# Wionerlol/MultimodalEmotionRecognition

Measured on AMD Instinct MI355X. Metric: 3s-clip train steps/sec (B=32, xattn fusion) at 1/2/4/8 MI355X, higher is better.
Workload: dtype bf16; 1 GPU; ResNet18 + WavLM-base (frozen) + xattn fusion train step (fwd+bwd+Adam); per_gpu_batch=32, global_batch=32, frames=8, image=112, audio_samples=48000, parallelism=dp1

## Files before the change

multimodalemotionrecognition_amd/csrc/conv.hip:

```cpp
#include "conv_common.h"
#include "mer.h"

MER_CT_BUFFER(mer_ct, 512 * 64)
MER_CT_BUFFER(mer_ctp, 4096 * 8)
#define CT(k) CT_AT(mer_ct_buf, k)
#define CTP(k) CTP_AT(mer_ctp_buf, k)

namespace {

template <bool DGRAD>
__device__ __forceinline__ u32x4 conv_a_chunk(const ConvGeom& g, int n, int oh, int ow, bool rowok, int kk, int tap,
                                              int c, int r, int s) {
  u32x4 v = {0u, 0u, 0u, 0u};
  if (!rowok || kk >= g.Kred) return v;
  int ih, iw;
  if (!DGRAD) {
    ih = oh * g.st - g.pad + r;
    iw = ow * g.st - g.pad + s;
  } else {
    const int th = oh + g.pad - r, tw = ow + g.pad - s;
    if (th < 0 || tw < 0) return v;
    if (g.st == 1) {
      ih = th;
      iw = tw;
    } else if (g.st == 2) {
      if ((th | tw) & 1) return v;
      ih = th >> 1;
      iw = tw >> 1;
    } else {
      if ((th % g.st) || (tw % g.st)) return v;
      ih = th / g.st;
      iw = tw / g.st;
    }
  }
  if (ih < 0 || ih >= g.IH || iw < 0 || iw >= g.IW) return v;
  return *reinterpret_cast<const u32x4*>(g.X + (((long)n * g.IH + ih) * g.IW + iw) * g.IC + c);
}

template <bool DGRAD, int BM_, int BN_>
__global__ __launch_bounds__(256, 2) void conv_kernel(ConvGeom g) {
  constexpr int LDK = CBK + 8;
  constexpr int IT = BM_ / 32, JT = BN_ / 32;
  constexpr int ACH = BM_ * 8 / 256, BCH = BN_ * 8 / 256;
  __shared__ __attribute__((aligned(16))) bf16_t lds[2][(BM_ + BN_) * LDK];
  const int t = threadIdx.x, lane = t & 63, w = t >> 6;
  const int M = g.N * g.OH * g.OW;
  const int nx = (g.Ncols + BN_ - 1) / BN_, ny = (M + BM_ - 1) / BM_;
  int tx, ty;
  xcd_tile(blockIdx.x, nx, nx * ny, tx, ty);
  const int m0 = ty * BM_, n0 = tx * BN_;
  const int wm = (w >> 1) * (BM_ / 2), wn = (w & 1) * (BN_ / 2);
  const int crow = t >> 3, ckc = t & 7;

  int an[ACH], aoh[ACH], aow[ACH];
  bool aok[ACH];
#pragma unroll
  for (int i = 0; i < ACH; ++i) {
    const int m = m0 + crow + 32 * i;
    aok[i] = m < M;
    const int mm = aok[i] ? m : 0;
    an[i] = mm / (g.OH * g.OW);
    const int rem = mm - an[i] * g.OH * g.OW;
    aoh[i] = rem / g.OW;
    aow[i] = rem - aoh[i] * g.OW;
  }
  u32x4 ra[ACH], rb[BCH];
  const float inv_IC = 1.f / g.IC, inv_S = 1.f / g.S;
  auto gload = [&](int k0) {
    const int kk = k0 + ckc * 8;
    const int tap = fdiv(kk, inv_IC), c = kk - tap * g.IC;
    const int r = fdiv(tap, inv_S), s = tap - r * g.S;
#pragma unroll
    for (int i = 0; i < ACH; ++i) ra[i] = conv_a_chunk<DGRAD>(g, an[i], aoh[i], aow[i], aok[i], kk, tap, c, r, s);
#pragma unroll
    for (int i = 0; i < BCH; ++i) {
      const int n = n0 + crow + 32 * i;
      rb[i] = (n < g.Ncols && kk < g.Kred) ? *reinterpret_cast<const u32x4*>(g.Wt + (long)n * g.Kred + kk)
                                            : u32x4{0u, 0u, 0u, 0u};
    }
  };
  auto lstore = [&](int buf) {
#pragma unroll
    for (int i = 0; i < ACH; ++i)
      *reinterpret_cast<u32x4*>(&lds[buf][(crow + 32 * i) * LDK + ckc * 8]) = ra[i];
#pragma unroll
    for (int i = 0; i < BCH; ++i)
      *reinterpret_cast<u32x4*>(&lds[buf][(BM_ + crow + 32 * i) * LDK + ckc * 8]) = rb[i];
  };
  f32x4 acc[IT][JT];
#pragma unroll
  for (int i = 0; i < IT; ++i)
#pragma unroll
    for (int j = 0; j < JT; ++j) acc[i][j] = f32x4{0.f, 0.f, 0.f, 0.f};

  const int nk = (g.Kred + CBK - 1) / CBK;
  gload(0);
  lstore(0);
  __syncthreads();
  for (int kt = 0; kt < nk; ++kt) {
    const int cur = kt & 1;
    if (kt + 1 < nk) gload((kt + 1) * CBK);
#pragma unroll
    for (int s = 0; s < 2; ++s) {
      const int kof = s * 32 + (lane >> 4) * 8;
      bf16x8 af[IT], bfr[JT];
#pragma unroll
      for (int i = 0; i < IT; ++i)
        af[i] = *reinterpret_cast<const bf16x8*>(&lds[cur][(wm + i * 16 + (lane & 15)) * LDK + kof]);
#pragma unroll
      for (int j = 0; j < JT; ++j)
        bfr[j] = *reinterpret_cast<const bf16x8*>(&lds[cur][(BM_ + wn + j * 16 + (lane & 15)) * LDK + kof]);
#pragma unroll
      for (int i = 0; i < IT; ++i)
#pragma unroll
        for (int j = 0; j < JT; ++j) acc[i][j] = __builtin_amdgcn_mfma_f32_16x16x32_bf16(af[i], bfr[j], acc[i][j], 0, 0, 0);
    }
    if (kt + 1 < nk) lstore(cur ^ 1);
    __syncthreads();
  }

#pragma unroll
  for (int j = 0; j < JT; ++j) {
    const int col = n0 + wn + j * 16 + (lane & 15);
    float csum = 0.f, csq = 0.f;
#pragma unroll
    for (int i = 0; i < IT; ++i)
#pragma unroll
      for (int r = 0; r < 4; ++r) {
        const int row = m0 + wm + i * 16 + (lane >> 4) * 4 + r;
        if (row < M && col < g.Ncols) {
          float v = acc[i][j][r];
          if (g.R_) {
            const long ri = (long)row * g.ldy + col;
            if (!g.Rmask || bf2f(g.Rmask[ri]) > 0.f) v += bf2f(g.R_[ri]);
          }
          const bf16_t h = f2bf(v);
          g.Y[(long)row * g.ldy + col] = h;
          const float hv = bf2f(h);
          csum += hv;
          csq += hv * hv;
        }
      }
    if (g.stats) {
      csum += __shfl_xor(csum, 16, 64);
      csum += __shfl_xor(csum, 32, 64);
      csq += __shfl_xor(csq, 16, 64);
      csq += __shfl_xor(csq, 32, 64);
      if ((lane >> 4) == 0 && col < g.Ncols) {
        float* slab = g.stats + (long)ty * g.Ncols * 2;
        atomicAdd(slab + 2 * col, csum);
        atomicAdd(slab + 2 * col + 1, csq);
      }
    }
  }
}


__device__ __forceinline__ int cswz(int row, int c) { return c ^ ((row >> 1) & 7); }
template <int CW>
__device__ __forceinline__ int cswz_k(int row, int c) {
  return CW == 8 ? (c ^ ((row >> 1) & 7)) : (c ^ ((row >> 2) & 3));
}

template <bool DGRAD>
__device__ __forceinline__ const bf16_t* conv_a_src(const ConvGeom& g, int n, int oh, int ow, bool rowok, int kk,
                                                    float inv_IC, float inv_S) {
  const bf16_t* zero = reinterpret_cast<const bf16_t*>(mer_conv_zero16);
  if (!rowok || kk >= g.Kred) return zero;
  const int tap = fdiv(kk, inv_IC), c = kk - tap * g.IC;
  const int r = fdiv(tap, inv_S), s = tap - r * g.S;
  int ih, iw;
  if (!DGRAD) {
    ih = oh * g.st - g.pad + r;
    iw = ow * g.st - g.pad + s;
  } else {
    const int th = oh + g.pad - r, tw = ow + g.pad - s;
    if (th < 0 || tw < 0) return zero;
    if (g.st == 1) {
      ih = th;
      iw = tw;
    } else {
      if ((th | tw) & 1) return zero;
      ih = th >> 1;
      iw = tw >> 1;
    }
  }
  if (ih < 0 || ih >= g.IH || iw < 0 || iw >= g.IW) return zero;
  return g.X + (((long)n * g.IH + ih) * g.IW + iw) * g.IC + c;
}

struct ParClass {
  int ph, pw, Hc, Wc, r0, s0, nr, ns, dh0, dw0;
};

__device__ __forceinline__ int par_cls() { return 3 - (int)blockIdx.y; }

__device__ __forceinline__ ParClass par_class(const ConvGeom& g, int cls) {
  ParClass c;
  c.ph = cls >> 1;
  c.pw = cls & 1;
  c.Hc = (g.OH - c.ph + 1) >> 1;
  c.Wc = (g.OW - c.pw + 1) >> 1;
  c.r0 = (c.ph + g.pad) & 1;
  c.s0 = (c.pw + g.pad) & 1;
  c.nr = (g.R - c.r0 + 1) >> 1;
  c.ns = (g.S - c.s0 + 1) >> 1;
  c.dh0 = (c.ph + g.pad - c.r0) >> 1;
  c.dw0 = (c.pw + g.pad - c.s0) >> 1;
  return c;
}

template <int FM, int FN, int WM, int WN>
__device__ __forceinline__ void conv_tile_stats_lane(const ConvGeom& g, const f32x4 (&acc)[FM][FN], int w, int lane,
                                                     int m0, int n0, int M, float (&part)[FN][2]) {
  constexpr int TM = FM * 16, TN = FN * 16;
  const int wr = w / WN, wc = w % WN, fr = lane & 15, fq = lane >> 4;
#pragma unroll
  for (int j = 0; j < FN; ++j) {
    const int col = n0 + wc * TN + j * 16 + fr;
    float csum = 0.f, csq = 0.f;
#pragma unroll
    for (int i = 0; i < FM; ++i)
#pragma unroll
      for (int r = 0; r < 4; ++r) {
        const int row = m0 + wr * TM + i * 16 + fq * 4 + r;
        if (row < M && col < g.Ncols) {
          const float hv = acc[i][j][r];
          csum += hv;
          csq += hv * hv;
        }
      }
    part[j][0] = csum;
    part[j][1] = csq;
  }
}

template <int FN, int WM, int WN>
__device__ __forceinline__ void conv_stats_finish(const ConvGeom& g, float (&part)[FN][2], float* red, int w, int lane,
                                                  int n0, long stat_row) {
  constexpr int TN = FN * 16;
  const int wr = w / WN, wc = w % WN, fr = lane & 15, fq = lane >> 4;
#pragma unroll
  for (int j = 0; j < FN; ++j)
#pragma unroll
    for (int q = 0; q < 2; ++q) {
      part[j][q] += __shfl_xor(part[j][q], 16, 64);
      part[j][q] += __shfl_xor(part[j][q], 32, 64);
    }
  lds_barrier();
  if (wr > 0 && fq == 0)
#pragma unroll
    for (int j = 0; j < FN; ++j) {
      red[((wr * WN + wc) * FN * 16 + j * 16 + fr) * 2] = part[j][0];
      red[((wr * WN + wc) * FN * 16 + j * 16 + fr) * 2 + 1] = part[j][1];
    }
  lds_barrier();
  if (wr == 0 && fq == 0) {
    float* slab = g.stats + stat_row * g.Ncols * 2;
#pragma unroll
    for (int j = 0; j < FN; ++j) {
      const int col = n0 + wc * TN + j * 16 + fr;
      float t0 = part[j][0], t1 = part[j][1];
#pragma unroll
      for (int q = 1; q < WM; ++q) {
        t0 += red[((q * WN + wc) * FN * 16 + j * 16 + fr) * 2];
        t1 += red[((q * WN + wc) * FN * 16 + j * 16 + fr) * 2 + 1];
      }
      if (col < g.Ncols) {
        slab[2 * col] = t0;
        slab[2 * col + 1] = t1;
      }
    }
  }
}

template <int FM, int FN, int WM, int WN>
__device__ __forceinline__ void conv_tile_stats(const ConvGeom& g, const f32x4 (&acc)[FM][FN], float* red, int w,
                                                int lane, int m0, int n0, int M, long stat_row) {
  float part[FN][2];
  conv_tile_stats_lane<FM, FN, WM, WN>(g, acc, w, lane, m0, n0, M, part);
  conv_stats_finish<FN, WM, WN>(g, part, red, w, lane, n0, stat_row);
}

typedef __attribute__((ext_vector_type(8))) float f32x8;
template <int FN>
struct EpiAcc {
  f32x8 sA, sB, sC;
  float fs[FN][2];
  __device__ void zero() {
    sA = sB = sC = f32x8{0.f, 0.f, 0.f, 0.f, 0.f, 0.f, 0.f, 0.f};
#pragma unroll
    for (int j = 0; j < FN; ++j) fs[j][0] = fs[j][1] = 0.f;
  }
};
struct EpiNoAcc {};

template <int FM, int FN, int WAVE_FLOATS>
struct EpiGeo {
  static constexpr int TM = FM * 16, TN = FN * 16, LDT = TN + 4;
  static constexpr int GI0 = WAVE_FLOATS / (16 * LDT);
  static constexpr int GI = GI0 < FM ? GI0 : FM;
  static constexpr int LPR = TN / 8, RPP = 64 / LPR;
  static constexpr int PPG = (GI * 16 + RPP - 1) / RPP;
  static constexpr int NP = ((FM + GI - 1) / GI) * PPG;
};

template <int NP>
struct EpiPre {
  u32x4 r[NP], m[NP], bm[NP], x[NP], x2[NP];
  float mu[8], rs[8], mu2[8], rs2[8];
};
struct EpiNone {};

template <bool DGRAD, int FM, int FN, int WM, int WN, int WAVE_FLOATS, class OutRow, int NP, bool X2 = true>
__device__ __forceinline__ void conv_epilogue_prefetch(const ConvGeom& g, EpiPre<NP>& pre, int w, int lane, int m0,
                                                       int n0, int M, OutRow out_row) {
  using E = EpiGeo<FM, FN, WAVE_FLOATS>;
  static_assert(NP == E::NP, "prefetch pass count");
  const int wr = w / WN, wc = w % WN;
  const int lr = lane / E::LPR, lc = (lane % E::LPR) * 8;
  const int colv = n0 + wc * E::TN + lc;
  const bool cok = colv < g.Ncols;
  const bool do_bnr = DGRAD && g.bnr_red != nullptr;
  const bool has_x2 = X2 && do_bnr && g.bnr_x2 != nullptr;
  const u32x4 z = {0u, 0u, 0u, 0u};
#pragma unroll
  for (int e = 0; e < 8; ++e) {
    const int col = cok ? colv + e : 0;
    pre.mu[e] = do_bnr ? g.bnr_ms[2 * col] : 0.f;
    pre.rs[e] = do_bnr ? g.bnr_ms[2 * col + 1] : 0.f;
    pre.mu2[e] = has_x2 ? g.bnr_ms2[2 * col] : 0.f;
    pre.rs2[e] = has_x2 ? g.bnr_ms2[2 * col + 1] : 0.f;
  }
#pragma unroll
  for (int q = 0; q < NP; ++q) {
    const int i0 = (q / E::PPG) * E::GI, rr = (q % E::PPG) * E::RPP;
    int row = m0 + wr * E::TM + i0 * 16 + rr + lr;
    row = row < M ? row : M - 1;
    const long e0 = out_row(row) * g.ldy + (cok ? colv : 0);
    pre.r[q] = (DGRAD && g.R_) ? *reinterpret_cast<const u32x4*>(g.R_ + e0) : z;
    pre.m[q] = (DGRAD && g.R_ && g.Rmask) ? *reinterpret_cast<const u32x4*>(g.Rmask + e0) : z;
    pre.bm[q] = do_bnr ? *reinterpret_cast<const u32x4*>(g.bnr_mask + e0) : z;
    pre.x[q] = do_bnr ? *reinterpret_cast<const u32x4*>(g.bnr_x + e0) : z;
    pre.x2[q] = has_x2 ? *reinterpret_cast<const u32x4*>(g.bnr_x2 + e0) : z;
  }
}

template <bool DGRAD, int FM, int FN, int WM, int WN, int WAVE_FLOATS, class OutRow, class Pre = EpiNone,
          bool DEFER = false, bool X2 = true, class AccT = EpiNoAcc>
__device__ __forceinline__ void conv_epilogue_vec(const ConvGeom& g, f32x4 (&acc)[FM][FN], float* smemf, int w,
                                                  int lane, int m0, int n0, int M, long red_row_id, long stat_row,
                                                  OutRow out_row, const Pre* pre = nullptr, int ct_slot = -1,
                                                  AccT* accp = nullptr) {
  constexpr bool PREF = !std::is_same<Pre, EpiNone>::value;
  constexpr bool ACC = !std::is_same<AccT, EpiNoAcc>::value;
  using E = EpiGeo<FM, FN, WAVE_FLOATS>;
  constexpr int TM = FM * 16, TN = FN * 16;
  const int wr = w / WN, wc = w % WN, fr = lane & 15, fq = lane >> 4;
  constexpr int LDT = TN + 4;
  constexpr int GI = E::GI;
  static_assert(GI >= 1, "epilogue staging slice too small");
  constexpr int LPR = TN / 8, RPP = 64 / LPR;
  float* wl = smemf + w * WAVE_FLOATS;
  const int lr = lane / LPR, lc = (lane % LPR) * 8;
  const int colv = n0 + wc * TN + lc;
  const bool cok = colv < g.Ncols;
  const bool do_bnr = DGRAD && g.bnr_red != nullptr;
  const bool has_x2 = X2 && do_bnr && g.bnr_x2 != nullptr;
  float mu[8], rs[8], mu2[8], rs2[8];
  float sA[8], sB[8], sC[8];
  constexpr int NPS = DEFER ? E::NP : 1;
  u32x4 pend[NPS];
  long pend_at[NPS];
  bool pend_ok[NPS];
#pragma unroll
  for (int q = 0; q < NPS; ++q) pend_ok[q] = false;
  auto flush = [&]() {
#pragma unroll
    for (int q = 0; q < NPS; ++q)
      if (pend_ok[q]) *reinterpret_cast<u32x4*>(g.Y + pend_at[q]) = pend[q];
  };
#pragma unroll
  for (int e = 0; e < 8; ++e) {
    if constexpr (PREF) {
      mu[e] = pre->mu[e];
      rs[e] = pre->rs[e];
      mu2[e] = pre->mu2[e];
      rs2[e] = pre->rs2[e];
    } else {
      const int col = cok ? colv + e : 0;
      mu[e] = do_bnr ? g.bnr_ms[2 * col] : 0.f;
      rs[e] = do_bnr ? g.bnr_ms[2 * col + 1] : 0.f;
      mu2[e] = has_x2 ? g.bnr_ms2[2 * col] : 0.f;
      rs2[e] = has_x2 ? g.bnr_ms2[2 * col + 1] : 0.f;
    }
    sA[e] = sB[e] = sC[e] = 0.f;
  }
#pragma unroll
  for (int i0 = 0; i0 < FM; i0 += GI) {
#pragma unroll
    for (int ii = 0; ii < GI; ++ii) {
      if (i0 + ii >= FM) break;
#pragma unroll
      for (int j = 0; j < FN; ++j)
#pragma unroll
        for (int r = 0; r < 4; ++r) wl[(ii * 16 + fq * 4 + r) * LDT + j * 16 + fr] = acc[i0 + ii][j][r];
    }
    __builtin_amdgcn_fence(__ATOMIC_RELEASE, "wavefront");
    __builtin_amdgcn_wave_barrier();
    __builtin_amdgcn_fence(__ATOMIC_ACQUIRE, "wavefront");
    const int nrows = (FM - i0 < GI ? FM - i0 : GI) * 16;
#pragma unroll
    for (int rr = 0; rr < GI * 16; rr += RPP) {
      const int rl = rr + lr;
      const int row = m0 + wr * TM + i0 * 16 + rl;
      if (rl < nrows && row < M && cok) {
        const f32x4 lo = *reinterpret_cast<const f32x4*>(&wl[rl * LDT + lc]);
        const f32x4 hi = *reinterpret_cast<const f32x4*>(&wl[rl * LDT + lc + 4]);
        float v[8] = {lo[0], lo[1], lo[2], lo[3], hi[0], hi[1], hi[2], hi[3]};
        const long e0 = out_row(row) * g.ldy + colv;
        const int q = (i0 / GI) * E::PPG + rr / RPP;
        if (DGRAD && g.R_) {
          u32x4 rv, mv;
          if constexpr (PREF) {
            rv = pre->r[q];
            mv = g.Rmask ? pre->m[q] : u32x4{1u, 1u, 1u, 1u};
          } else {
            rv = *reinterpret_cast<const u32x4*>(g.R_ + e0);
            mv = g.Rmask ? *reinterpret_cast<const u32x4*>(g.Rmask + e0) : u32x4{1u, 1u, 1u, 1u};
          }
          const bf16_t* rh = reinterpret_cast<const bf16_t*>(&rv);
          const bf16_t* mh = reinterpret_cast<const bf16_t*>(&mv);
#pragma unroll
          for (int e = 0; e < 8; ++e)
            if (!g.Rmask || bf2f(mh[e]) > 0.f) v[e] += bf2f(rh[e]);
        }
        u32x4 ov;
        bf16_t* oh = reinterpret_cast<bf16_t*>(&ov);
#pragma unroll
        for (int e = 0; e < 8; ++e) {
          oh[e] = f2bf(v[e]);
          v[e] = bf2f(oh[e]);
        }
        if constexpr (DEFER) {
          pend[q] = ov;
          pend_at[q] = e0;
          pend_ok[q] = true;
        } else {
          *reinterpret_cast<u32x4*>(g.Y + e0) = ov;
        }
        if (do_bnr) {
          u32x4 mv, xv, x2v;
          if constexpr (PREF) {
            mv = pre->bm[q];
            xv = pre->x[q];
            x2v = pre->x2[q];
          } else {
            mv = *reinterpret_cast<const u32x4*>(g.bnr_mask + e0);
            xv = *reinterpret_cast<const u32x4*>(g.bnr_x + e0);
            x2v = has_x2 ? *reinterpret_cast<const u32x4*>(g.bnr_x2 + e0) : u32x4{0u, 0u, 0u, 0u};
          }
          const bf16_t* mh = reinterpret_cast<const bf16_t*>(&mv);
          const bf16_t* xh = reinterpret_cast<const bf16_t*>(&xv);
          const bf16_t* x2h = reinterpret_cast<const bf16_t*>(&x2v);
#pragma unroll
          for (int e = 0; e < 8; ++e) {
            const float gv = bf2f(mh[e]) > 0.f ? v[e] : 0.f;
            sA[e] += gv;
            sB[e] += gv * (bf2f(xh[e]) - mu[e]) * rs[e];
            if (has_x2) sC[e] += gv * (bf2f(x2h[e]) - mu2[e]) * rs2[e];
          }
        }
      }
    }
    __builtin_amdgcn_fence(__ATOMIC_RELEASE, "wavefront");
    __builtin_amdgcn_wave_barrier();
    __builtin_amdgcn_fence(__ATOMIC_ACQUIRE, "wavefront");
  }
  if (ct_slot >= 0) CT(ct_slot);
  if constexpr (ACC) {
    if (do_bnr) {
#pragma unroll
      for (int e = 0; e < 8; ++e) {
        accp->sA[e] += sA[e];
        accp->sB[e] += sB[e];
        accp->sC[e] += sC[e];
      }
      flush();
      return;
    }
  }
  if (do_bnr) {
#pragma unroll
  for (int o = LPR; o < 64; o <<= 1)
#pragma unroll
    for (int e = 0; e < 8; ++e) {
      sA[e] += __shfl_xor(sA[e], o, 64);
      sB[e] += __shfl_xor(sB[e], o, 64);
      if (has_x2) sC[e] += __shfl_xor(sC[e], o, 64);
    }
  if (ct_slot >= 0) CT(ct_slot + 3);
  float* red = smemf;
  lds_barrier();
  if (ct_slot >= 0) CT(ct_slot + 4);
  if (wr > 0 && lane < LPR)
#pragma unroll
    for (int e = 0; e < 8; ++e) {
      float* o = red + ((wr * WN + wc) * TN + lc + e) * 3;
      o[0] = sA[e];
      o[1] = sB[e];
      o[2] = sC[e];
    }
  lds_barrier();
  if (wr != 0 || lane >= LPR || !cok) {
    flush();
    return;
  }
#pragma unroll
  for (int e = 0; e < 8; ++e)
#pragma unroll
    for (int q = 1; q < WM; ++q) {
      const float* o = red + ((q * WN + wc) * TN + lc + e) * 3;
      sA[e] += o[0];
      sB[e] += o[1];
      sC[e] += o[2];
    }
  {
    const long slab = red_row_id * g.Ncols * 2 + 2 * colv;
#pragma unroll
    for (int e = 0; e < 8; e += 2) {
      *reinterpret_cast<f32x4*>(g.bnr_red + slab + 2 * e) = f32x4{sA[e], sB[e], sA[e + 1], sB[e + 1]};
      if (g.bnr_red2)
        *reinterpret_cast<f32x4*>(g.bnr_red2 + slab + 2 * e) = f32x4{sA[e], sC[e], sA[e + 1], sC[e + 1]};
    }
  }
  if (ct_slot >= 0) CT(ct_slot + 1);
  flush();
  if (ct_slot >= 0) CT(ct_slot + 2);
  return;
  }
  if (!g.stats) {
    flush();
    return;
  }
#pragma unroll
  for (int i = 0; i < FM; ++i)
#pragma unroll
    for (int j = 0; j < FN; ++j)
#pragma unroll
      for (int r = 0; r < 4; ++r) acc[i][j][r] = bf2f(f2bf(acc[i][j][r]));
  if constexpr (ACC) {
    float part[FN][2];
    conv_tile_stats_lane<FM, FN, WM, WN>(g, acc, w, lane, m0, n0, M, part);
#pragma unroll
    for (int j = 0; j < FN; ++j) {
      accp->fs[j][0] += part[j][0];
      accp->fs[j][1] += part[j][1];
    }
    flush();
    return;
  }
  conv_tile_stats<FM, FN, WM, WN>(g, acc, smemf, w, lane, m0, n0, M, stat_row);
  if (ct_slot >= 0) CT(ct_slot + 1);
  flush();
  if (ct_slot >= 0) CT(ct_slot + 2);
}

template <bool DGRAD, int FM, int FN, int WM, int WN, int WAVE_FLOATS, bool X2 = true>
__device__ __forceinline__ void conv_epilogue_acc_finish(const ConvGeom& g, EpiAcc<FN>& a, float* smemf, int w,
                                                         int lane, int n0, long row_id) {
  if constexpr (DGRAD) {
    if (!g.bnr_red) return;
    using E = EpiGeo<FM, FN, WAVE_FLOATS>;
    constexpr int TN = FN * 16, LPR = E::LPR;
    const int wr = w / WN, wc = w % WN;
    const int lc = (lane % LPR) * 8;
    const int colv = n0 + wc * TN + lc;
    const bool cok = colv < g.Ncols;
    const bool has_x2 = X2 && g.bnr_x2 != nullptr;
#pragma unroll
    for (int o = LPR; o < 64; o <<= 1)
#pragma unroll
      for (int e = 0; e < 8; ++e) {
        a.sA[e] += __shfl_xor(a.sA[e], o, 64);
        a.sB[e] += __shfl_xor(a.sB[e], o, 64);
        if (has_x2) a.sC[e] += __shfl_xor(a.sC[e], o, 64);
      }
    float* red = smemf;
    lds_barrier();
    if (wr > 0 && lane < LPR)
#pragma unroll
      for (int e = 0; e < 8; ++e) {
        float* o = red + ((wr * WN + wc) * TN + lc + e) * 3;
        o[0] = a.sA[e];
        o[1] = a.sB[e];
        o[2] = a.sC[e];
      }
    lds_barrier();
    if (wr != 0 || lane >= LPR || !cok) return;
#pragma unroll
    for (int e = 0; e < 8; ++e)
#pragma unroll
      for (int q = 1; q < WM; ++q) {
        const float* o = red + ((q * WN + wc) * TN + lc + e) * 3;
        a.sA[e] += o[0];
        a.sB[e] += o[1];
        a.sC[e] += o[2];
      }
    const long slab = row_id * g.Ncols * 2 + 2 * colv;
#pragma unroll
    for (int e = 0; e < 8; e += 2) {
      *reinterpret_cast<f32x4*>(g.bnr_red + slab + 2 * e) = f32x4{a.sA[e], a.sB[e], a.sA[e + 1], a.sB[e + 1]};
      if (g.bnr_red2)
        *reinterpret_cast<f32x4*>(g.bnr_red2 + slab + 2 * e) = f32x4{a.sA[e], a.sC[e], a.sA[e + 1], a.sC[e + 1]};
    }
  } else {
    if (!g.stats) return;
    conv_stats_finish<FN, WM, WN>(g, a.fs, smemf, w, lane, n0, row_id);
  }
}

constexpr int conv_pipe_wpe(int nw, int bm, int bn, int stages, bool dgrad, bool par, int lds_bytes = 0) {
  return (nw >= 16 || 2 * lds_bytes > 160 * 1024)
             ? (nw >= 4 ? nw / 4 : 1)
             : nw == 8 ? ((dgrad && (bm == 256 || (!par && bm == 128 && bn == 128 && stages == 3))) ? 2 : 4) : 2;
}
constexpr int conv_pipe_lds(int bm, int bn, int stages, int ks, int kg) {
  return kg * stages * (bm + bn) * ks * 2 > (kg > 1 ? kg * bm * (bn + 4) * 4 : 0)
             ? kg * stages * (bm + bn) * ks * 2
             : kg * bm * (bn + 4) * 4;
}

template <int BM_, int BN_, int NW>
struct KgLayout {
  static constexpr int WM = (NW >= 4 && BM_ / 4 >= 16) ? 4 : (NW >= 2 ? 2 : 1);
  static constexpr int WN = NW / WM;
  static_assert(WM * WN == NW && BM_ % (16 * WM) == 0 && BN_ % (16 * WN) == 0, "split-K epilogue layout");
};

template <bool DGRAD, bool PAR, int BM_, int BN_, int WM = 2, int WN = 2, int STAGES = 2, int KS = 64, bool X2 = true,
          int KG = 1, bool FAST = false>
__global__ __launch_bounds__(64 * WM * WN * KG, conv_pipe_wpe(WM * WN * KG, BM_, BN_, STAGES, DGRAD, PAR,
                                                              conv_pipe_lds(BM_, BN_, STAGES, KS, KG))) void conv_pipe_kernel(ConvGeom g) {
  constexpr int WAVES = WM * WN;
  constexpr int CW = KS / 8, RPG = 64 / CW;
  constexpr int IA = BM_ / RPG / WAVES, IB = BN_ / RPG / WAVES;
  static_assert(IA * RPG * WAVES == BM_ && IB * RPG * WAVES == BN_, "tile rows must split into whole glds pieces");
  static_assert(KS == 64 || KS == 32, "K-tile");
  static_assert(KG == 1 || KG == 2 || KG == 4, "K-groups");
  constexpr int TM = BM_ / WM, TN = BN_ / WN, FM = TM / 16, FN = TN / 16;
  constexpr int BUF = (BM_ + BN_) * KS;
  extern __shared__ __attribute__((aligned(16))) bf16_t smem_all[];
  const int t = threadIdx.x, lane = t & 63, kg = (t >> 6) / WAVES, w = (t >> 6) % WAVES;
  bf16_t* const smem = smem_all + kg * STAGES * BUF;
  ParClass pc{};
  int M, Kr, rowsH, rowsW;
  int Kr0 = 0;
  if (PAR) {
    pc = par_class(g, par_cls());
    M = g.N * pc.Hc * pc.Wc;
    Kr0 = pc.nr * pc.ns * g.IC;
    Kr = Kr0 + ((g.X2 && pc.ph == 0 && pc.pw == 0) ? g.K2 : 0);
    rowsH = pc.Hc;
    rowsW = pc.Wc;
  } else {
    M = g.N * g.OH * g.OW;
    Kr = g.Kred;
    rowsH = g.OH;
    rowsW = g.OW;
  }
  const int nx = (g.Ncols + BN_ - 1) / BN_, ny = (M + BM_ - 1) / BM_;
  if ((int)blockIdx.x >= nx * ny) return;
  CTP(0);
  int tx, ty;
  xcd_tile(blockIdx.x, nx, nx * ny, tx, ty);
  const int m0 = ty * BM_, n0 = tx * BN_;
  const int wr = w / WN, wc = w % WN;

  auto a_row = [&](int j, int& n, int& oh, int& ow, bool& ok) {
    const int m = m0 + (w * IA + j) * RPG + lane / CW;
    ok = m < M;
    const int mm = ok ? m : 0;
    n = mm / (rowsH * rowsW);
    const int rem = mm - n * rowsH * rowsW;
    oh = rem / rowsW;
    ow = rem - oh * rowsW;
  };
  int acl[IA];
#pragma unroll
  for (int j = 0; j < IA; ++j) acl[j] = cswz_k<CW>((w * IA + j) * RPG + lane / CW, lane % CW) * 8;
  int bcl[IB], bn[IB];
  bool bok[IB];
#pragma unroll
  for (int j = 0; j < IB; ++j) {
    const int r = (w * IB + j) * RPG + lane / CW;
    const int n = n0 + r;
    bok[j] = n < g.Ncols;
    bn[j] = bok[j] ? n : 0;
    bcl[j] = cswz_k<CW>(r, lane % CW) * 8;
  }
  const bf16_t* zero = reinterpret_cast<const bf16_t*>(mer_conv_zero16);

  f32x4 acc[FM][FN];
#pragma unroll
  for (int i = 0; i < FM; ++i)
#pragma unroll
    for (int j = 0; j < FN; ++j) acc[i][j] = f32x4{0.f, 0.f, 0.f, 0.f};

  const int fr = lane & 15, fq = lane >> 4;
  const int nk_all = (Kr + KS - 1) / KS;
  const int nkg = (nk_all + KG - 1) / KG, kb = __builtin_amdgcn_readfirstlane(kg * nkg);
  const int nk = nk_all - kb < nkg ? (nk_all - kb > 0 ? nk_all - kb : 0) : nkg;
  const int kofs = kb * KS;
  constexpr int G = IA + IB;
  static_assert(STAGES >= 2 && STAGES <= 4, "ring depth");
  auto k_loop = [&](auto&& stage) {
#pragma unroll
    for (int p = 0; p < STAGES - 1; ++p)
      if (p < nk) stage(p);
    int wslot = STAGES - 1, rslot = 0;
    CTP(1);
    for (int kt = 0; kt < nkg; ++kt) {
      const int left = nk - 1 - kt;
      const int ahead = left < (STAGES - 2) ? left : (STAGES - 2);
      wait_tiles_in_flight<G>(ahead);
      lds_barrier();
      if (kt + STAGES - 1 < nk) stage(wslot);
      wslot = wslot == STAGES - 1 ? 0 : wslot + 1;
      const bf16_t* la = smem + rslot * BUF;
      rslot = rslot == STAGES - 1 ? 0 : rslot + 1;
      if (KG > 1 && kt >= nk) continue;
      const bf16_t* lb = la + BM_ * KS;
#pragma unroll
      for (int s = 0; s < KS / 32; ++s) {
        bf16x8 af[FM], bfr[FN];
#pragma unroll
        for (int i = 0; i < FM; ++i) {
          const int r = wr * TM + i * 16 + fr;
          af[i] = *reinterpret_cast<const bf16x8*>(la + r * KS + cswz_k<CW>(r, s * 4 + fq) * 8);
        }
#pragma unroll
        for (int j = 0; j < FN; ++j) {
          const int r = wc * TN + j * 16 + fr;
          bfr[j] = *reinterpret_cast<const bf16x8*>(lb + r * KS + cswz_k<CW>(r, s * 4 + fq) * 8);
        }
        __builtin_amdgcn_s_setprio(1);
#pragma unroll
        for (int i = 0; i < FM; ++i)
#pragma unroll
          for (int j = 0; j < FN; ++j)
            acc[i][j] = __builtin_amdgcn_mfma_f32_16x16x32_bf16(af[i], bfr[j], acc[i][j], 0, 0, 0);
        __builtin_amdgcn_s_setprio(0);
      }
    }
  };

  if constexpr (FAST) {
    const bool has_ds = PAR && Kr > Kr0;
    constexpr bool NEG = DGRAD || PAR;
    const int nr = PAR ? pc.nr : g.R, ns = PAR ? pc.ns : g.S;
    const bf16_t* fa[IA];
    unsigned fm[IA];
#pragma unroll
    for (int j = 0; j < IA; ++j) {
      int n, oh, ow;
      bool ok;
      a_row(j, n, oh, ow, ok);
      const int h0 = PAR ? oh + pc.dh0 : DGRAD ? oh + g.pad : oh * g.st - g.pad;
      const int w0 = PAR ? ow + pc.dw0 : DGRAD ? ow + g.pad : ow * g.st - g.pad;
      unsigned cm = 0, m = 0;
      for (int si = 0; si < ns; ++si) cm |= (unsigned)((unsigned)(NEG ? w0 - si : w0 + si) < (unsigned)g.IW) << si;
      for (int ri = 0; ri < nr; ++ri)
        if ((unsigned)(NEG ? h0 - ri : h0 + ri) < (unsigned)g.IH) m |= cm << (ri * ns);
      fm[j] = ok ? m : 0u;
      fa[j] = g.X + ((((long)n * g.IH + h0) * g.IW + w0) * g.IC + acl[j]);
    }
    const bf16_t* fb[IB];
#pragma unroll
    for (int j = 0; j < IB; ++j) fb[j] = g.Wt + ((long)bn[j] * g.Kred + bcl[j]);
    int f_ic = g.IC, f_c, f_tap, f_ri, f_si, f_aoff, f_boff;
    bool f_ds = false;
    auto tap_offsets = [&]() {
      const int ao = (f_ri * g.IW + f_si) * g.IC;
      f_aoff = NEG ? -ao : ao;
      f_boff = PAR ? ((pc.r0 + 2 * f_ri) * g.S + pc.s0 + 2 * f_si) * g.IC : f_tap * g.IC;
    };
    auto enter_ds = [&]() {
      f_ds = true;
      f_ic = g.K2;
      f_c = f_tap = f_ri = f_si = f_aoff = f_boff = 0;
#pragma unroll
      for (int j = 0; j < IA; ++j) {
        int n, hh, ww;
        bool ok;
        a_row(j, n, hh, ww, ok);
        fm[j] = ok ? 1u : 0u;
        fa[j] = g.X2 + ((((long)n * g.IH + hh) * g.IW + ww) * g.K2 + acl[j]);
      }
#pragma unroll
      for (int j = 0; j < IB; ++j) fb[j] = g.Wt2 + ((long)bn[j] * g.K2 + bcl[j]);
    };
    if (has_ds && kofs >= Kr0) {
      enter_ds();
      f_c = kofs - Kr0;
    } else {
      f_tap = kofs / g.IC;
      f_c = kofs - f_tap * g.IC;
      f_ri = f_tap / (ns > 0 ? ns : 1);
      f_si = f_tap - f_ri * ns;
      tap_offsets();
    }
    k_loop([&](int buf) {
      bf16_t* la = smem + buf * BUF;
      bf16_t* lb = la + BM_ * KS;
      const unsigned tbit = 1u << (f_tap & 31);
      const long ao = f_aoff + f_c, bo = f_boff + f_c;
#pragma unroll
      for (int j = 0; j < IA; ++j) glds16((fm[j] & tbit) ? fa[j] + ao : zero, la + (w * IA + j) * 512);
#pragma unroll
      for (int j = 0; j < IB; ++j) glds16(bok[j] ? fb[j] + bo : zero, lb + (w * IB + j) * 512);
      f_c += KS;
      if (f_c == f_ic) {
        f_c = 0;
        ++f_tap;
        if (++f_si == ns) {
          f_si = 0;
          ++f_ri;
        }
        tap_offsets();
        if (has_ds && !f_ds && f_tap == nr * ns) enter_ds();
      }
    });
  } else {
    int an[IA], aoh[IA], aow[IA];
    bool aok[IA];
#pragma unroll
    for (int j = 0; j < IA; ++j) a_row(j, an[j], aoh[j], aow[j], aok[j]);
    const bf16_t* pb[IB];
    const bf16_t* pb2[IB];
#pragma unroll
    for (int j = 0; j < IB; ++j) {
      pb[j] = g.Wt + (long)bn[j] * g.Kred;
      pb2[j] = g.Wt2 + (long)bn[j] * g.K2;
    }
    const float inv_IC = 1.f / g.IC, inv_S = 1.f / g.S, inv_ns = PAR ? 1.f / pc.ns : 1.f;
    auto par_a_src = [&](int n, int hh, int ww, bool rowok, int kk) -> const bf16_t* {
      if (!rowok || kk >= Kr) return zero;
      if (kk >= Kr0)
        return g.X2 + (((long)n * g.IH + hh) * g.IW + ww) * g.K2 + (kk - Kr0);
      const int tap = fdiv(kk, inv_IC), c = kk - tap * g.IC;
      const int ri = fdiv(tap, inv_ns), si = tap - ri * pc.ns;
      const int ih = hh + pc.dh0 - ri, iw = ww + pc.dw0 - si;
      if (ih < 0 || ih >= g.IH || iw < 0 || iw >= g.IW) return zero;
      return g.X + (((long)n * g.IH + ih) * g.IW + iw) * g.IC + c;
    };
    auto par_b_off = [&](int kk) -> int {
      const int tap = fdiv(kk, inv_IC), c = kk - tap * g.IC;
      const int ri = fdiv(tap, inv_ns), si = tap - ri * pc.ns;
      return ((pc.r0 + 2 * ri) * g.S + pc.s0 + 2 * si) * g.IC + c;
    };
    int k0 = kofs;
    k_loop([&](int buf) {
      bf16_t* la = smem + buf * BUF;
      bf16_t* lb = la + BM_ * KS;
#pragma unroll
      for (int j = 0; j < IA; ++j) {
        const bf16_t* src = PAR ? par_a_src(an[j], aoh[j], aow[j], aok[j], k0 + acl[j])
                                : conv_a_src<DGRAD>(g, an[j], aoh[j], aow[j], aok[j], k0 + acl[j], inv_IC, inv_S);
        glds16(src, la + (w * IA + j) * 512);
      }
#pragma unroll
      for (int j = 0; j < IB; ++j) {
        const int kk = k0 + bcl[j];
        const bool ok = bok[j] && kk < Kr;
        const bf16_t* src = !PAR ? pb[j] + kk : (kk >= Kr0 ? pb2[j] + (kk - Kr0) : pb[j] + par_b_off(kk));
        glds16(ok ? src : zero, lb + (w * IB + j) * 512);
      }
      k0 += KS;
    });
  }
  CTP(2);

  auto out_row = [&](int row) -> long {
    if (!PAR) return (long)row;
    const int n = row / (pc.Hc * pc.Wc);
    const int rem = row - n * pc.Hc * pc.Wc;
    const int hh = rem / pc.Wc, ww = rem - hh * pc.Wc;
    return ((long)n * g.OH + 2 * hh + pc.ph) * g.OW + 2 * ww + pc.pw;
  };
  auto red_row = [&]() -> long {
    long row_id = ty;
    if (PAR)
      for (int c2 = 0; c2 < par_cls(); ++c2) {
        const ParClass q = par_class(g, c2);
        row_id += (g.N * q.Hc * q.Wc + BM_ - 1) / BM_;
      }
    return row_id;
  };
  constexpr int EWF = STAGES * BUF / 2 / WAVES;
  const int ct_slot = 10;
  if constexpr (KG > 1) {
    using L = KgLayout<BM_, BN_, WAVES * KG>;
    constexpr int LDR = BN_ + 4;
    constexpr int TM2 = BM_ / L::WM, TN2 = BN_ / L::WN, FM2 = TM2 / 16, FN2 = TN2 / 16;
    using E2 = EpiGeo<FM2, FN2, EWF>;
    const int w2 = t >> 6, wr2 = w2 / L::WN, wc2 = w2 % L::WN;
    constexpr bool PF = DGRAD && E2::NP == 1;
    EpiPre<E2::NP> pre;
    if constexpr (PF)
      conv_epilogue_prefetch<DGRAD, FM2, FN2, L::WM, L::WN, EWF, decltype(out_row), E2::NP, X2>(g, pre, w2, lane, m0,
                                                                                                n0, M, out_row);
    __syncthreads();
    float* const part = reinterpret_cast<float*>(smem_all);
    {
      float* mine = part + kg * BM_ * LDR;
#pragma unroll
      for (int i = 0; i < FM; ++i)
#pragma unroll
        for (int j = 0; j < FN; ++j)
#pragma unroll
          for (int r = 0; r < 4; ++r) mine[(wr * TM + i * 16 + fq * 4 + r) * LDR + wc * TN + j * 16 + fr] = acc[i][j][r];
    }
    lds_barrier();
    f32x4 acc2[FM2][FN2];
#pragma unroll
    for (int i = 0; i < FM2; ++i)
#pragma unroll
      for (int j = 0; j < FN2; ++j)
#pragma unroll
        for (int r = 0; r < 4; ++r) {
          const int e = (wr2 * TM2 + i * 16 + fq * 4 + r) * LDR + wc2 * TN2 + j * 16 + fr;
          float s = part[e];
#pragma unroll
          for (int q = 1; q < KG; ++q) s += part[q * BM_ * LDR + e];
          acc2[i][j][r] = s;
        }
    lds_barrier();
    CTP(3);
    if constexpr (PF)
      conv_epilogue_vec<DGRAD, FM2, FN2, L::WM, L::WN, EWF, decltype(out_row), decltype(pre), false, X2>(
          g, acc2, reinterpret_cast<float*>(smem_all), w2, lane, m0, n0, M, g.bnr_red ? red_row() : 0l, ty, out_row,
          &pre, ct_slot);
    else
      conv_epilogue_vec<DGRAD, FM2, FN2, L::WM, L::WN, EWF, decltype(out_row), EpiNone, false, X2>(
          g, acc2, reinterpret_cast<float*>(smem_all), w2, lane, m0, n0, M, (DGRAD && g.bnr_red) ? red_row() : 0l, ty,
          out_row, static_cast<const EpiNone*>(nullptr), ct_slot);
    CTP(4);
    return;
  }
  if (g.vec) {
    using E1 = EpiGeo<FM, FN, EWF>;
    if constexpr (DGRAD && E1::NP == 1) {
      EpiPre<E1::NP> pre;
      conv_epilogue_prefetch<DGRAD, FM, FN, WM, WN, EWF, decltype(out_row), E1::NP, X2>(g, pre, w, lane, m0, n0, M,
                                                                                         out_row);
      __syncthreads();
      CTP(3);
      conv_epilogue_vec<DGRAD, FM, FN, WM, WN, EWF, decltype(out_row), decltype(pre), false, X2>(
          g, acc, reinterpret_cast<float*>(smem), w, lane, m0, n0, M, g.bnr_red ? red_row() : 0l, ty, out_row, &pre,
          ct_slot);
    } else {
      __syncthreads();
      CTP(3);
      conv_epilogue_vec<DGRAD, FM, FN, WM, WN, EWF, decltype(out_row), EpiNone, false, X2>(
          g, acc, reinterpret_cast<float*>(smem), w, lane, m0, n0, M, (DGRAD && g.bnr_red) ? red_row() : 0l, ty,
          out_row, static_cast<const EpiNone*>(nullptr), ct_slot);
    }
    CTP(4);
    return;
  } else {
  __syncthreads();
#pragma unroll
  for (int i = 0; i < FM; ++i)
#pragma unroll
    for (int r = 0; r < 4; ++r) {
      const int row = m0 + wr * TM + i * 16 + fq * 4 + r;
      if (row >= M) continue;
      const long orow = out_row(row) * g.ldy;
#pragma unroll
      for (int j = 0; j < FN; ++j) {
        const int col = n0 + wc * TN + j * 16 + fr;
        if (col >= g.Ncols) continue;
        float v = acc[i][j][r];
        if (g.R_) {
          const long ri = orow + col;
          if (!g.Rmask || bf2f(g.Rmask[ri]) > 0.f) v += bf2f(g.R_[ri]);
        }
        const bf16_t h = f2bf(v);
        g.Y[orow + col] = h;
        acc[i][j][r] = bf2f(h);
      }
    }
  if (DGRAD && g.bnr_red) {
    float ps[FN][3];
#pragma unroll
    for (int j = 0; j < FN; ++j) {
      const int col = n0 + wc * TN + j * 16 + fr;
      const bool cok = col < g.Ncols;
      const float mu = cok ? g.bnr_ms[2 * col] : 0.f, rs = cok ? g.bnr_ms[2 * col + 1] : 0.f;
      const float mu2 = (cok && g.bnr_x2) ? g.bnr_ms2[2 * col] : 0.f;
      const float rs2 = (cok && g.bnr_x2) ? g.bnr_ms2[2 * col + 1] : 0.f;
      float s1 = 0.f, s2 = 0.f, s3 = 0.f;
#pragma unroll
      for (int i = 0; i < FM; ++i)
#pragma unroll
        for (int r = 0; r < 4; ++r) {
          const int row = m0 + wr * TM + i * 16 + fq * 4 + r;
          if (row < M && cok) {
            const long e = out_row(row) * g.ldy + col;
            const float gv = bf2f(g.bnr_mask[e]) > 0.f ? acc[i][j][r] : 0.f;
            s1 += gv;
            s2 += gv * (bf2f(g.bnr_x[e]) - mu) * rs;
            if (g.bnr_x2) s3 += gv * (bf2f(g.bnr_x2[e]) - mu2) * rs2;
          }
        }
#pragma unroll
      for (int o = 16; o < 64; o <<= 1) {
        s1 += __shfl_xor(s1, o, 64);
        s2 += __shfl_xor(s2, o, 64);
        s3 += __shfl_xor(s3, o, 64);
      }
      ps[j][0] = s1;
      ps[j][1] = s2;
      ps[j][2] = s3;
    }
    float* red = reinterpret_cast<float*>(smem);
    __syncthreads();
    if (wr > 0 && fq == 0)
#pragma unroll
      for (int j = 0; j < FN; ++j)
#pragma unroll
        for (int q = 0; q < 3; ++q) red[((wr * WN + wc) * FN * 16 + j * 16 + fr) * 3 + q] = ps[j][q];
    __syncthreads();
    if (wr == 0 && fq == 0) {
      long row_id = ty;
      if (PAR)
        for (int c2 = 0; c2 < par_cls(); ++c2) {
          const ParClass q = par_class(g, c2);
          row_id += (g.N * q.Hc * q.Wc + BM_ - 1) / BM_;
        }
      const long slab = row_id * g.Ncols * 2;
#pragma unroll
      for (int j = 0; j < FN; ++j) {
        const int col = n0 + wc * TN + j * 16 + fr;
        float t0 = ps[j][0], t1 = ps[j][1], t2 = ps[j][2];
#pragma unroll
        for (int q = 1; q < WM; ++q) {
          const float* o = red + ((q * WN + wc) * FN * 16 + j * 16 + fr) * 3;
          t0 += o[0];
          t1 += o[1];
          t2 += o[2];
        }
        if (col < g.Ncols) {
          g.bnr_red[slab + 2 * col] = t0;
// ... 476 lines not shown
```

Measured before the change: 225.2 steps/s.

## Issue all LDS fragment reads up front in conv k-loop with explicit lgkmcnt waits

The conv pipeline's inner K loop now issues every sub-step's A/B fragment reads at the start of each K tile. It does this with inline ds_read_b128 using immediate offsets, then waits on lgkmcnt before each MFMA group, so the reads for later sub-steps overlap the earlier MFMAs. With deeper rings (STAGES>2), the next tile's global-to-LDS stage is issued after the fragment reads rather than before. The wave index and zero pointer are also forced into scalar registers. The trade-offs are higher VGPR pressure from holding all fragments at once, and the correctness of the hand-counted lgkmcnt values depends on what else the stage issues.

```diff
diff --git a/multimodalemotionrecognition_amd/csrc/conv.hip b/multimodalemotionrecognition_amd/csrc/conv.hip
--- a/multimodalemotionrecognition_amd/csrc/conv.hip
+++ b/multimodalemotionrecognition_amd/csrc/conv.hip
@@ -160,6 +160,29 @@
 template <int CW>
 __device__ __forceinline__ int cswz_k(int row, int c) {
   return CW == 8 ? (c ^ ((row >> 1) & 7)) : (c ^ ((row >> 2) & 3));
+}
+
+template <int OFF>
+__device__ __forceinline__ bf16x8 frag_read(const bf16_t* p) {
+  static_assert(OFF >= 0 && OFF < 65536, "ds offset field");
+  typedef __attribute__((address_space(3))) const char lds_cchar;
+  const uint32_t a = (uint32_t)(uintptr_t)(lds_cchar*)p;
+  bf16x8 v;
+  asm volatile("ds_read_b128 %0, %1 offset:%2" : "=v"(v) : "v"(a), "n"(OFF) : "memory");
+  return v;
+}
+template <int N>
+__device__ __forceinline__ void frag_wait() {
+  static_assert(N >= 0 && N < 16, "lgkmcnt range");
+  asm volatile("s_waitcnt lgkmcnt(%0)" ::"n"(N) : "memory");
+}
+__device__ __forceinline__ void frag_ready(bf16x8& f) { asm volatile("" : "+v"(f)); }
+template <int I, int N, class F>
+__device__ __forceinline__ void static_for(F&& f) {
+  if constexpr (I < N) {
+    f(std::integral_constant<int, I>{});
+    static_for<I + 1, N>(f);
+  }
 }
 
 template <bool DGRAD>
@@ -651,7 +674,9 @@
   constexpr int TM = BM_ / WM, TN = BN_ / WN, FM = TM / 16, FN = TN / 16;
   constexpr int BUF = (BM_ + BN_) * KS;
   extern __shared__ __attribute__((aligned(16))) bf16_t smem_all[];
-  const int t = threadIdx.x, lane = t & 63, kg = (t >> 6) / WAVES, w = (t >> 6) % WAVES;
+  const int t = threadIdx.x, lane = t & 63;
+  const int wv = __builtin_amdgcn_readfirstlane(t >> 6);
+  const int kg = wv / WAVES, w = wv % WAVES;
   bf16_t* const smem = smem_all + kg * STAGES * BUF;
   ParClass pc{};
   int M, Kr, rowsH, rowsW;
@@ -700,6 +725,7 @@
     bcl[j] = cswz_k<CW>(r, lane % CW) * 8;
   }
   const bf16_t* zero = reinterpret_cast<const bf16_t*>(mer_conv_zero16);
+  asm volatile("" : "+s"(zero));
 
   f32x4 acc[FM][FN];
 #pragma unroll
@@ -713,6 +739,7 @@
   const int nk = nk_all - kb < nkg ? (nk_all - kb > 0 ? nk_all - kb : 0) : nkg;
   const int kofs = kb * KS;
   constexpr int G = IA + IB;
+  constexpr int NSUB = KS / 32;
   static_assert(STAGES >= 2 && STAGES <= 4, "ring depth");
   auto k_loop = [&](auto&& stage) {
 #pragma unroll
@@ -725,31 +752,44 @@
       const int ahead = left < (STAGES - 2) ? left : (STAGES - 2);
       wait_tiles_in_flight<G>(ahead);
       lds_barrier();
-      if (kt + STAGES - 1 < nk) stage(wslot);
+      if (KG > 1 && kt >= nk) continue;
+      constexpr bool READS_FIRST = STAGES > 2;
+      if constexpr (!READS_FIRST) {
+        if (kt + STAGES - 1 < nk) stage(wslot);
+        __builtin_amdgcn_sched_barrier(0);
+      }
+      const bf16_t* la = smem + rslot * BUF;
+      const bf16_t* lb = la + BM_ * KS;
+      rslot = rslot == STAGES - 1 ? 0 : rslot + 1;
+      bf16x8 af[NSUB][FM], bfr[NSUB][FN];
+#pragma unroll
+      for (int s = 0; s < NSUB; ++s) {
+        const int ra = wr * TM + fr, rb = wc * TN + fr;
+        const bf16_t* pa = la + ra * KS + cswz_k<CW>(ra, s * 4 + fq) * 8;
+        const bf16_t* pb = lb + rb * KS + cswz_k<CW>(rb, s * 4 + fq) * 8;
+        static_for<0, FM>([&](auto i) { af[s][decltype(i)::value] = frag_read<decltype(i)::value * 16 * KS * 2>(pa); });
+        static_for<0, FN>([&](auto j) { bfr[s][decltype(j)::value] = frag_read<decltype(j)::value * 16 * KS * 2>(pb); });
+      }
+      __builtin_amdgcn_sched_barrier(0);
+      if constexpr (READS_FIRST) {
+        if (kt + STAGES - 1 < nk) stage(wslot);
+        __builtin_amdgcn_sched_barrier(0);
+      }
       wslot = wslot == STAGES - 1 ? 0 : wslot + 1;
-      const bf16_t* la = smem + rslot * BUF;
-      rslot = rslot == STAGES - 1 ? 0 : rslot + 1;
-      if (KG > 1 && kt >= nk) continue;
-      const bf16_t* lb = la + BM_ * KS;
-#pragma unroll
-      for (int s = 0; s < KS / 32; ++s) {
-        bf16x8 af[FM], bfr[FN];
-#pragma unroll
-        for (int i = 0; i < FM; ++i) {
-          const int r = wr * TM + i * 16 + fr;
-          af[i] = *reinterpret_cast<const bf16x8*>(la + r * KS + cswz_k<CW>(r, s * 4 + fq) * 8);
-        }
-#pragma unroll
-        for (int j = 0; j < FN; ++j) {
-          const int r = wc * TN + j * 16 + fr;
-          bfr[j] = *reinterpret_cast<const bf16x8*>(lb + r * KS + cswz_k<CW>(r, s * 4 + fq) * 8);
-        }
+#pragma unroll
+      for (int s = 0; s < NSUB; ++s) {
+        if (s + 1 < NSUB) frag_wait<(NSUB - 1) * (FM + FN)>();
+        else frag_wait<0>();
+#pragma unroll
+        for (int i = 0; i < FM; ++i) frag_ready(af[s][i]);
+#pragma unroll
+        for (int j = 0; j < FN; ++j) frag_ready(bfr[s][j]);
         __builtin_amdgcn_s_setprio(1);
 #pragma unroll
         for (int i = 0; i < FM; ++i)
 #pragma unroll
           for (int j = 0; j < FN; ++j)
-            acc[i][j] = __builtin_amdgcn_mfma_f32_16x16x32_bf16(af[i], bfr[j], acc[i][j], 0, 0, 0);
+            acc[i][j] = __builtin_amdgcn_mfma_f32_16x16x32_bf16(af[s][i], bfr[s][j], acc[i][j], 0, 0, 0);
         __builtin_amdgcn_s_setprio(0);
       }
     }
```

Result: no change. 225.3 steps/s, median of 5 (+0.0%).
